# ithewei/libhv

Hardware: AMD Instinct MI355X
Metric: device-resident WS unmask GiB/s, 64 KiB masked frames, 1/2/4/8 MI355X (higher is better)
Workload: dtype u8

## Files before the change

### libhv_amd/csrc/hvws_utf8.hip

```cpp
#include "hvws_dev.h"

namespace hvws {

namespace {

constexpr int U8_T = 256, U8_U = 4;
static_assert((uint64_t)U8_T * U8_U * 16u == U8_TILE, "tile geometry");
constexpr int U8_MAXF = 512;

__device__ __forceinline__ uint32_t u8_step(uint32_t s, uint32_t b) {
    if (s == 0u) {
        if (b < 0x80u) return 0u;
        if (b < 0xC2u) return U8_REJECT;
        if (b < 0xE0u) return 1u;
        if (b == 0xE0u) return 3u;
        if (b == 0xEDu) return 4u;
        if (b < 0xF0u) return 2u;
        if (b == 0xF0u) return 5u;
        if (b < 0xF4u) return 6u;
        return b == 0xF4u ? 7u : U8_REJECT;
    }
    if (s > 7u) return U8_REJECT;
    const uint32_t lo = s == 3u ? 0xA0u : (s == 5u ? 0x90u : 0x80u);
    const uint32_t hi = s == 4u ? 0x9Fu : (s == 7u ? 0x8Fu : 0xBFu);
    if (b < lo || b > hi) return U8_REJECT;
    return s == 1u ? 0u : (s <= 4u ? 1u : 2u);
}

__device__ __forceinline__ uint32_t u8_len(uint32_t b) {
    return b < 0x80u ? 1u : b < 0xC0u ? 0u : b < 0xC2u ? 9u : b < 0xE0u ? 2u : b < 0xF0u ? 3u : b < 0xF5u ? 4u : 9u;
}

__device__ __forceinline__ bool u8_ok2(uint32_t p, uint32_t q) {
    const uint32_t lo = p == 0xE0u ? 0xA0u : (p == 0xF0u ? 0x90u : 0x80u);
    const uint32_t hi = p == 0xEDu ? 0x9Fu : (p == 0xF4u ? 0x8Fu : 0xBFu);
    return q >= lo && q <= hi;
}

__device__ __forceinline__ bool u8_chunk_bad(const u32x4 w, const uint32_t h, const uint32_t jlo,
                                             const uint32_t jhi) {
    if (((w.x | w.y | w.z | w.w | (h >> 8)) & 0x80808080u) == 0u) return false;
    {
        auto top4 = [](uint32_t x) { return (((x >> 7) & 0x01010101u) * 0x01020408u) >> 24; };
        const uint32_t hb = (top4(h) >> 1) | (top4(w.x) << 3) | (top4(w.y) << 7) | (top4(w.z) << 11) | (top4(w.w) << 15);
        const uint32_t reads = ((1u << (jhi + 3u)) - 1u) & ~((1u << jlo) - 1u);
        if ((hb & reads) == 0u) return false;
    }
    uint32_t B[19], L[19];
    B[0] = (h >> 8) & 0xFFu;
    B[1] = (h >> 16) & 0xFFu;
    B[2] = h >> 24;
    const uint32_t ww[4] = {w.x, w.y, w.z, w.w};
#pragma unroll
    for (int q = 0; q < 16; ++q) B[3 + q] = (ww[q >> 2] >> (8 * (q & 3))) & 0xFFu;
#pragma unroll
    for (int q = 0; q < 19; ++q) L[q] = u8_len(B[q]);
    bool P[18];
#pragma unroll
    for (int q = 0; q < 18; ++q) P[q] = u8_ok2(B[q], B[q + 1]);
    uint32_t badm = 0u;
#pragma unroll
    for (int j = 0; j < 16; ++j) {
        const uint32_t l0 = L[j + 3], l1 = L[j + 2], l2 = L[j + 1], l3 = L[j];
        bool ok;
        if (l0 == 0u)
            ok = l1 != 0u ? (l1 >= 2u && l1 <= 4u && P[j + 2])
               : l2 != 0u ? (l2 >= 3u && l2 <= 4u && P[j + 1])
               : l3 != 0u ? (l3 == 4u && P[j])
                          : false;
        else
            ok = l0 != 9u && (l1 != 0u ? l1 == 1u : l2 != 0u ? l2 == 2u : l3 != 0u ? (l3 == 3u && P[j]) : true);
        badm |= ok ? 0u : (1u << j);
    }
    const uint32_t act = (jhi >= 16u ? 0xFFFFu : ((1u << jhi) - 1u)) & ~((1u << jlo) - 1u);
    return (badm & act) != 0u;
}

__device__ __forceinline__ void u8_report(bool bad, uint32_t rec, uint32_t* __restrict__ flags) {
    uint64_t m = __ballot(bad);
    const uint32_t lane = threadIdx.x & 63u;
    while (m) {
        const int l = __ffsll((unsigned long long)m) - 1;
        const uint32_t r = (uint32_t)__shfl((int)rec, l);
        const uint64_t same = __ballot(bad && rec == r);
        if (lane == (uint32_t)l) atomicOr(&flags[r], 1u);
        m &= ~same;
    }
}

template <typename OFF, typename END, typename KEY>
__device__ __forceinline__ void u8_chunk(const u32x4 v, const uint32_t h, const uint64_t c, const uint32_t k0,
                                         const uint32_t nf, OFF offf, END endf, KEY keyf, bool& bad, uint32_t& brec,
                                         uint32_t* __restrict__ flags) {
    uint32_t lo = 0, hi = nf;
    while (lo < hi) {
        const uint32_t mid = (lo + hi) >> 1;
        if (endf(mid) > c) hi = mid;
        else lo = mid + 1;
    }
#pragma unroll 1
    for (uint32_t k = lo; k < nf; ++k) {
        const uint64_t o = offf(k), e = endf(k);
        if (o >= c + 16) break;
        const uint64_t from = o + 3 > c ? o + 3 - c : 0;
        const uint32_t jlo = from > 16 ? 16u : (uint32_t)from;
        const uint32_t jhi = e < c + 16 ? (e > c ? (uint32_t)(e - c) : 0u) : 16u;
        if (jlo < jhi) {
            const uint32_t kw = keyf(k);
            if (u8_chunk_bad(v ^ u32x4{kw, kw, kw, kw}, h ^ kw, jlo, jhi)) {
                if (!bad) {
                    bad = true;
                    brec = k0 + k;
                } else if (brec != k0 + k) {
                    atomicOr(&flags[k0 + k], 1u);
                }
            }
        }
        if (e > c + 16) break;
    }
}

__global__ __launch_bounds__(U8_T) void k_u8_tiles(const uint8_t* __restrict__ rx, uint64_t rx_len,
                                                   const uint64_t* __restrict__ pay_off,
                                                   const uint64_t* __restrict__ pay_len,
                                                   const uint32_t* __restrict__ keyrot,
                                                   const uint32_t* __restrict__ tile_first,
                                                   const uint64_t* __restrict__ nfr_p, uint64_t cap, uint32_t masked,
                                                   uint32_t* __restrict__ flags) {
    constexpr int T = U8_T, U = U8_U;
    __shared__ uint64_t s_off[U8_MAXF];
    __shared__ uint64_t s_end[U8_MAXF];
    __shared__ uint32_t s_key[U8_MAXF];

    const uint64_t t = blockIdx.x;
    const uint64_t base = t * U8_TILE;
    const uint32_t tid = threadIdx.x;
    const uint64_t nfr = *nfr_p < cap ? *nfr_p : cap;
    const uint32_t k0 = tile_first[t];
    const uint32_t k1r = tile_first[t + 1];
    const uint32_t k1 = (uint64_t)k1r + 1 < nfr ? k1r + 1 : (uint32_t)nfr;
    const uint32_t nf = k1 > k0 ? k1 - k0 : 0u;
    if (nf == 0u) return;

    const bool full = base + U8_TILE <= rx_len;
    u32x4 v[U];
    uint32_t h[U];
#pragma unroll
    for (int i = 0; i < U; ++i) {
        const uint64_t c = base + ((uint64_t)i * T + tid) * 16u;
        if (full || c + 16 <= rx_len) {
            v[i] = *reinterpret_cast<const u32x4*>(rx + c);
        } else {
            uint32_t w[4] = {0u, 0u, 0u, 0u};
            for (int b = 0; b < 16; ++b)
                if (c + b < rx_len) w[b >> 2] |= (uint32_t)rx[c + b] << (8 * (b & 3));
            v[i] = u32x4{w[0], w[1], w[2], w[3]};
        }
    }
#pragma unroll
    for (int i = 0; i < U; ++i) {
        const uint64_t c = base + ((uint64_t)i * T + tid) * 16u;
        uint32_t prev = (uint32_t)__shfl_up((int)v[i].w, 1);
        if ((tid & 63u) == 0u) prev = (c >= 16 && c <= rx_len) ? *reinterpret_cast<const uint32_t*>(rx + c - 4) : 0u;
        h[i] = prev;
    }

    const bool staged = nf <= (uint32_t)U8_MAXF;
    if (staged) {
        for (uint32_t i = tid; i < nf; i += T) {
            const uint64_t o = pay_off[k0 + i], n = pay_len[k0 + i];
            s_off[i] = o;
            s_end[i] = n > 6 ? o + n : o;
            s_key[i] = masked ? keyrot[k0 + i] : 0u;
        }
    }
    __syncthreads();

#pragma unroll
    for (int i = 0; i < U; ++i) {
        const uint64_t c = base + ((uint64_t)i * T + tid) * 16u;
        bool bad = false;
        uint32_t brec = 0u;
        if (c < rx_len) {
            if (staged)
                u8_chunk(
                    v[i], h[i], c, k0, nf, [&](uint32_t k) { return s_off[k]; }, [&](uint32_t k) { return s_end[k]; },
                    [&](uint32_t k) { return s_key[k]; }, bad, brec, flags);
            else
                u8_chunk(
                    v[i], h[i], c, k0, nf, [&](uint32_t k) { return pay_off[k0 + k]; },
                    [&](uint32_t k) {
                        const uint64_t n = pay_len[k0 + k];
                        return n > 6 ? pay_off[k0 + k] + n : pay_off[k0 + k];
                    },
                    [&](uint32_t k) { return masked ? keyrot[k0 + k] : 0u; }, bad, brec, flags);
        }
        u8_report(bad, brec, flags);
    }
}

__global__ __launch_bounds__(256) void k_u8_words(const uint8_t* __restrict__ rx, uint64_t rx_len,
                                                  const uint64_t* __restrict__ pay_off,
                                                  const uint64_t* __restrict__ pay_len,
                                                  const uint32_t* __restrict__ keyrot,
                                                  const uint64_t* __restrict__ nfr_p, uint64_t cap, uint32_t masked,
                                                  uint32_t* __restrict__ flags, uint32_t* __restrict__ words,
                                                  uint64_t* __restrict__ meta) {
    const uint64_t nfr = *nfr_p < cap ? *nfr_p : cap;
    const uint64_t k = (uint64_t)blockIdx.x * blockDim.x + threadIdx.x;
    if (k == 0) meta[0] = nfr;
    if (k >= nfr) return;
    const uint64_t o = pay_off[k], n = pay_len[k];
    const uint32_t kw = masked ? keyrot[k] : 0u;
    const uint32_t interior_bad = flags[k];
    if (interior_bad) flags[k] = 0u;
    if (o > rx_len || n > rx_len - o) {
        words[k] = 0xFFFFFFFFu;
        return;
    }
    auto byte_at = [&](uint64_t i) -> uint32_t {
        const uint64_t a = o + i;
        return ((uint32_t)rx[a] ^ (kw >> (8u * (uint32_t)(a & 3u)))) & 0xFFu;
    };
    uint32_t word = 0u;
    if (n <= 6) {
        uint32_t d[6];
#pragma unroll
        for (int i = 0; i < 6; ++i) d[i] = (uint64_t)i < n ? byte_at(i) : 0u;
#pragma unroll
        for (uint32_t e = 0; e < 8; ++e) {
            uint32_t s = e;
#pragma unroll
            for (int i = 0; i < 6; ++i)
                if ((uint64_t)i < n) s = u8_step(s, d[i]);
            word |= s << (4u * e);
        }
    } else {
        const uint32_t d0 = byte_at(0), d1 = byte_at(1), d2 = byte_at(2);
        const uint32_t t0 = byte_at(n - 3), t1 = byte_at(n - 2), t2 = byte_at(n - 1);
        uint32_t tail = 0u;
        if (u8_len(t2) != 0u) tail = u8_step(0u, t2);
        else if (u8_len(t1) != 0u) tail = u8_step(u8_step(0u, t1), t2);
        else if (u8_len(t0) != 0u) tail = u8_step(u8_step(u8_step(0u, t0), t1), t2);
#pragma unroll
        for (uint32_t e = 0; e < 8; ++e) {
            const uint32_t s = u8_step(u8_step(u8_step(e, d0), d1), d2);
            word |= ((s == U8_REJECT || interior_bad) ? U8_REJECT : tail) << (4u * e);
        }
    }
    words[k] = word;
}

__device__ __forceinline__ void u8_apply(uint32_t& st, uint32_t& text, uint32_t inf, uint32_t w) {
    const uint32_t op = inf & F_OPMASK;
    if (op >= 3u) return;
    if ((inf & I_HDR) && op == 1u) {
        text = 1u;
        st = U8_ACCEPT;
    } else if ((inf & I_HDR) && op == 2u) {
        text = 0u;
        st = U8_ACCEPT;
    }
    if (text && (inf & I_BODY)) st = st > 7u ? U8_REJECT : (w >> (4u * st)) & 15u;
    if ((inf & I_END) && (inf & F_FIN) && text) {
        if (st != U8_ACCEPT) st = U8_REJECT;
        text = 0u;
    }
}

__global__ __launch_bounds__(256) void k_u8_fold(const uint32_t* __restrict__ info, const uint32_t* __restrict__ words,
                                                 const uint64_t* __restrict__ meta,
                                                 const uint64_t* __restrict__ counts,
                                                 const uint64_t* __restrict__ bases, uint32_t nseg,
                                                 const uint32_t* __restrict__ state_in,
                                                 uint32_t* __restrict__ state_out, uint64_t* __restrict__ bad_out) {
    const uint32_t s = __builtin_amdgcn_readfirstlane(blockIdx.x * (blockDim.x >> 6) + (threadIdx.x >> 6));
    if (s >= nseg) return;
    const uint32_t lane = threadIdx.x & 63u;
    const uint64_t nrec = meta[0];
    const uint64_t first = bases[s];
    uint64_t cnt = counts[s];
    if (first >= nrec) cnt = 0;
    else if (cnt > nrec - first) cnt = nrec - first;
    const uint32_t sw = state_in ? state_in[s] : 0u;
    uint32_t st = sw & 15u, text = (sw >> 4) & 1u;
    uint64_t bad = ~0ull;
    if (st > 7u) {
        st = U8_REJECT;
        bad = first;
        cnt = 0;
    }
    for (uint64_t b0 = 0; b0 < cnt && bad == ~0ull; b0 += 64) {
        const uint64_t left = cnt - b0;
        const uint32_t m = left < 64 ? (uint32_t)left : 64u;
        const uint32_t my_info = lane < m ? info[first + b0 + lane] : 8u;
        const uint32_t my_word = lane < m ? words[first + b0 + lane] : U8_IDENTITY;
        const uint32_t op = my_info & F_OPMASK;
        const bool reset = (my_info & I_HDR) && (op == 1u || op == 2u);
        const uint64_t below = __ballot(reset) & ((2ull << lane) - 1ull);
        const uint32_t r = below ? 63u - (uint32_t)__clzll((long long)below) : 0u;
        uint32_t lst = below ? U8_ACCEPT : st, ltext = below ? 0u : text;
        const uint32_t span = lane < m ? lane - r : 0u;
        for (uint32_t t = 0;; ++t) {
            const bool act = lane < m && t <= span;
            if (!__ballot(act)) break;
            const uint32_t src = r + t < 64u ? r + t : 63u;
            const uint32_t inf = (uint32_t)__shfl((int)my_info, (int)src);
            const uint32_t w = (uint32_t)__shfl((int)my_word, (int)src);
            if (act) u8_apply(lst, ltext, inf, w);
        }
        const uint64_t rej = __ballot(lane < m && lst == U8_REJECT);
        if (rej) {
            st = U8_REJECT;
            bad = first + b0 + (uint64_t)(__ffsll((unsigned long long)rej) - 1);
        } else {
            st = (uint32_t)__builtin_amdgcn_readlane((int)lst, (int)(m - 1u));
            text = (uint32_t)__builtin_amdgcn_readlane((int)ltext, (int)(m - 1u));
        }
    }
    if (st == U8_REJECT) text = 0u;
    if (lane == 0u) {
        state_out[s] = st | (text << 4);
        bad_out[s] = bad;
    }
}

}

hipError_t launch_utf8(const uint8_t* rx, uint64_t rx_len, const uint64_t* pay_off, const uint64_t* pay_len,
                       const uint32_t* keyrot, const uint32_t* info, const uint64_t* nfr_dev, uint64_t cap,
                       const uint32_t* tile_first, uint64_t ntiles, int masked, uint32_t* flags, uint32_t* words,
                       uint64_t* meta, const uint64_t* counts, const uint64_t* bases, uint32_t nseg,
                       const uint32_t* state_in, uint32_t* state_out, uint64_t* bad, hipStream_t st) {
    if (ntiles)
        hipLaunchKernelGGL(k_u8_tiles, dim3((uint32_t)ntiles), dim3(U8_T), 0, st, rx, rx_len, pay_off, pay_len, keyrot,
                           tile_first, nfr_dev, cap, masked ? 1u : 0u, flags);
    const uint64_t wb = (cap + 255) / 256;
    hipLaunchKernelGGL(k_u8_words, dim3((uint32_t)(wb ? wb : 1)), dim3(256), 0, st, rx, rx_len, pay_off, pay_len, keyrot,
                       nfr_dev, cap, masked ? 1u : 0u, flags, words, meta);
    if (nseg)
        hipLaunchKernelGGL(k_u8_fold, dim3((nseg + 3) / 4), dim3(256), 0, st, info, words, meta, counts, bases, nseg,
                           state_in, state_out, bad);
    return hipGetLastError();
}

}
```

Baseline: 3017.

## Replace per-byte UTF-8 check with SWAR predicate and single-frame fast path

Swaps the scalar 19-byte UTF-8 validation inside u8_chunk_bad for a SWAR bitwise classifier that works on whole 32-bit words, using alignbyte to shift across word boundaries. It also adds an early path for tiles that sit entirely inside one frame's payload: the XOR key is applied and every chunk is checked without staging frame metadata in shared memory or searching records. Both aim to cut ALU work and per-tile bookkeeping on the validation kernel. The cost is a complex, hard-to-verify bit-trick predicate that must match the reference exactly, and the early return skips the __syncthreads path for the whole block.

Result: slower. 2811 (-6.8%).

```diff
diff --git a/libhv_amd/csrc/hvws_u8_pred.h b/libhv_amd/csrc/hvws_u8_pred.h
--- /dev/null
+++ b/libhv_amd/csrc/hvws_u8_pred.h
@@ -0,0 +1,117 @@
+#pragma once
+#include <stdint.h>
+
+#if defined(__HIPCC__)
+#define HVWS_U8_FN __host__ __device__ __forceinline__
+#else
+#define HVWS_U8_FN inline
+#endif
+
+namespace hvws {
+
+HVWS_U8_FN uint32_t u8_len(uint32_t b) {
+    return b < 0x80u ? 1u : b < 0xC0u ? 0u : b < 0xC2u ? 9u : b < 0xE0u ? 2u : b < 0xF0u ? 3u : b < 0xF5u ? 4u : 9u;
+}
+
+HVWS_U8_FN bool u8_ok2(uint32_t p, uint32_t q) {
+    const uint32_t lo = p == 0xE0u ? 0xA0u : (p == 0xF0u ? 0x90u : 0x80u);
+    const uint32_t hi = p == 0xEDu ? 0x9Fu : (p == 0xF4u ? 0x8Fu : 0xBFu);
+    return q >= lo && q <= hi;
+}
+
+HVWS_U8_FN uint32_t u8_pred_ref(uint32_t w0, uint32_t w1, uint32_t w2, uint32_t w3, uint32_t h) {
+    uint32_t B[19], L[19];
+    B[0] = (h >> 8) & 0xFFu;
+    B[1] = (h >> 16) & 0xFFu;
+    B[2] = h >> 24;
+    const uint32_t ww[4] = {w0, w1, w2, w3};
+#pragma unroll
+    for (int q = 0; q < 16; ++q) B[3 + q] = (ww[q >> 2] >> (8 * (q & 3))) & 0xFFu;
+#pragma unroll
+    for (int q = 0; q < 19; ++q) L[q] = u8_len(B[q]);
+    bool P[18];
+#pragma unroll
+    for (int q = 0; q < 18; ++q) P[q] = u8_ok2(B[q], B[q + 1]);
+    uint32_t badm = 0u;
+#pragma unroll
+    for (int j = 0; j < 16; ++j) {
+        const uint32_t l0 = L[j + 3], l1 = L[j + 2], l2 = L[j + 1], l3 = L[j];
+        bool ok;
+        if (l0 == 0u)
+            ok = l1 != 0u ? (l1 >= 2u && l1 <= 4u && P[j + 2])
+               : l2 != 0u ? (l2 >= 3u && l2 <= 4u && P[j + 1])
+               : l3 != 0u ? (l3 == 4u && P[j])
+                          : false;
+        else
+            ok = l0 != 9u && (l1 != 0u ? l1 == 1u : l2 != 0u ? l2 == 2u : l3 != 0u ? (l3 == 3u && P[j]) : true);
+        badm |= ok ? 0u : (1u << j);
+    }
+    return badm;
+}
+
+HVWS_U8_FN uint32_t u8_bytes_from(uint32_t hi, uint32_t lo, uint32_t n) {
+#if defined(__HIP_DEVICE_COMPILE__)
+    return __builtin_amdgcn_alignbyte(hi, lo, n);
+#else
+    return (lo >> (8u * n)) | (hi << (32u - 8u * n));
+#endif
+}
+
+struct U8Cls {
+    uint32_t cc, w1, w2, w3, c, z;
+};
+
+HVWS_U8_FN U8Cls u8_classes(uint32_t x, uint32_t nx) {
+    constexpr uint32_t M = 0x80808080u, ONE = 0x01010101u;
+    const uint32_t y = x & 0x7F7F7F7Fu;
+    const uint32_t gC2 = y + 0x3Eu * ONE, gE0 = y + 0x20u * ONE, gE1 = y + 0x1Fu * ONE, gED = y + 0x13u * ONE,
+                   gEE = y + 0x12u * ONE, gF0 = y + 0x10u * ONE, gF1 = y + 0x0Fu * ONE, gF4 = y + 0x0Cu * ONE,
+                   gF5 = y + 0x0Bu * ONE;
+    const uint32_t n5 = nx << 2, n45 = n5 | (nx << 3);
+    const uint32_t e0 = gE0 & ~gE1, ed = gED & ~gEE, f0 = gF0 & ~gF1, f4 = gF4 & ~gF5;
+    const uint32_t fl = ((ed & n5) | (e0 & ~n5)) | ((f4 & n45) | (f0 & ~n45));
+    const uint32_t nf = x & ~(gF5 | fl);
+    const uint32_t u1 = nf & gC2, u2 = nf & gE0, u3 = nf & gF0;
+    const uint32_t xr = x >> 1;
+    const uint32_t c = x & ~(x << 1);
+    const uint32_t c6 = xr & ~x;
+    const uint32_t v3 = (u2 & ~gF0) | c;
+    const uint32_t l2 = x & gC2 & ~gE0;
+    U8Cls k;
+    k.cc = (c & M) | (c6 & ~M);
+    k.w1 = (u1 & M) | (~xr & ~M);
+    k.w2 = (u2 & M) | ((l2 >> 1) & ~M);
+    k.w3 = (u3 & M) | ((v3 >> 1) & ~M);
+    k.c = c;
+    k.z = x & ~(gC2 & ~gF5);
+    return k;
+}
+
+HVWS_U8_FN void u8_pred_flags(uint32_t w0, uint32_t w1, uint32_t w2, uint32_t w3, uint32_t h, uint32_t bad[4]) {
+    constexpr uint32_t M = 0x80808080u;
+    const uint32_t x[5] = {h, w0, w1, w2, w3};
+    U8Cls k[5];
+#pragma unroll
+    for (int i = 0; i < 5; ++i) k[i] = u8_classes(x[i], u8_bytes_from(i < 4 ? x[i + 1] : 0u, x[i], 1));
+    uint32_t y2[5], y1[5];
+#pragma unroll
+    for (int i = 0; i < 5; ++i) y2[i] = k[i].w2 | (k[i].cc & u8_bytes_from(k[i].w3, i ? k[i - 1].w3 : 0u, 3));
+#pragma unroll
+    for (int i = 0; i < 5; ++i) y1[i] = k[i].w1 | (k[i].cc & u8_bytes_from(y2[i], i ? y2[i - 1] : 0u, 3));
+#pragma unroll
+    for (int i = 1; i < 5; ++i) {
+        const uint32_t r = u8_bytes_from(y1[i], y1[i - 1], 3);
+        bad[i - 1] = M & ~((k[i].c & r) | ((r << 1) & ~k[i].z));
+    }
+}
+
+HVWS_U8_FN uint32_t u8_pred(uint32_t w0, uint32_t w1, uint32_t w2, uint32_t w3, uint32_t h) {
+    uint32_t bad[4];
+    u8_pred_flags(w0, w1, w2, w3, h, bad);
+    uint32_t r = 0u;
+#pragma unroll
+    for (int i = 0; i < 4; ++i) r |= (((bad[i] >> 7) * 0x01020408u) >> 24) << (4 * i);
+    return r;
+}
+
+}
diff --git a/libhv_amd/csrc/hvws_utf8.hip b/libhv_amd/csrc/hvws_utf8.hip
--- a/libhv_amd/csrc/hvws_utf8.hip
+++ b/libhv_amd/csrc/hvws_utf8.hip
@@ -1,4 +1,5 @@
 #include "hvws_dev.h"
+#include "hvws_u8_pred.h"
 
 namespace hvws {
 
@@ -27,16 +28,6 @@
     return s == 1u ? 0u : (s <= 4u ? 1u : 2u);
 }
 
-__device__ __forceinline__ uint32_t u8_len(uint32_t b) {
-    return b < 0x80u ? 1u : b < 0xC0u ? 0u : b < 0xC2u ? 9u : b < 0xE0u ? 2u : b < 0xF0u ? 3u : b < 0xF5u ? 4u : 9u;
-}
-
-__device__ __forceinline__ bool u8_ok2(uint32_t p, uint32_t q) {
-    const uint32_t lo = p == 0xE0u ? 0xA0u : (p == 0xF0u ? 0x90u : 0x80u);
-    const uint32_t hi = p == 0xEDu ? 0x9Fu : (p == 0xF4u ? 0x8Fu : 0xBFu);
-    return q >= lo && q <= hi;
-}
-
 __device__ __forceinline__ bool u8_chunk_bad(const u32x4 w, const uint32_t h, const uint32_t jlo,
                                              const uint32_t jhi) {
     if (((w.x | w.y | w.z | w.w | (h >> 8)) & 0x80808080u) == 0u) return false;
@@ -46,32 +37,7 @@
         const uint32_t reads = ((1u << (jhi + 3u)) - 1u) & ~((1u << jlo) - 1u);
         if ((hb & reads) == 0u) return false;
     }
-    uint32_t B[19], L[19];
-    B[0] = (h >> 8) & 0xFFu;
-    B[1] = (h >> 16) & 0xFFu;
-    B[2] = h >> 24;
-    const uint32_t ww[4] = {w.x, w.y, w.z, w.w};
-#pragma unroll
-    for (int q = 0; q < 16; ++q) B[3 + q] = (ww[q >> 2] >> (8 * (q & 3))) & 0xFFu;
-#pragma unroll
-    for (int q = 0; q < 19; ++q) L[q] = u8_len(B[q]);
-    bool P[18];
-#pragma unroll
-    for (int q = 0; q < 18; ++q) P[q] = u8_ok2(B[q], B[q + 1]);
-    uint32_t badm = 0u;
-#pragma unroll
-    for (int j = 0; j < 16; ++j) {
-        const uint32_t l0 = L[j + 3], l1 = L[j + 2], l2 = L[j + 1], l3 = L[j];
-        bool ok;
-        if (l0 == 0u)
-            ok = l1 != 0u ? (l1 >= 2u && l1 <= 4u && P[j + 2])
-               : l2 != 0u ? (l2 >= 3u && l2 <= 4u && P[j + 1])
-               : l3 != 0u ? (l3 == 4u && P[j])
-                          : false;
-        else
-            ok = l0 != 9u && (l1 != 0u ? l1 == 1u : l2 != 0u ? l2 == 2u : l3 != 0u ? (l3 == 3u && P[j]) : true);
-        badm |= ok ? 0u : (1u << j);
-    }
+    const uint32_t badm = u8_pred(w.x, w.y, w.z, w.w, h);
     const uint32_t act = (jhi >= 16u ? 0xFFFFu : ((1u << jhi) - 1u)) & ~((1u << jlo) - 1u);
     return (badm & act) != 0u;
 }
@@ -163,6 +129,18 @@
         uint32_t prev = (uint32_t)__shfl_up((int)v[i].w, 1);
         if ((tid & 63u) == 0u) prev = (c >= 16 && c <= rx_len) ? *reinterpret_cast<const uint32_t*>(rx + c - 4) : 0u;
         h[i] = prev;
+    }
+
+    if (nf == 1u && full) {
+        const uint64_t o = pay_off[k0], n = pay_len[k0];
+        if (n > 6 && o + 3 <= base && base + U8_TILE <= o + n) {
+            const uint32_t kw = masked ? keyrot[k0] : 0u;
+            bool bad = false;
+#pragma unroll
+            for (int i = 0; i < U; ++i) bad |= u8_chunk_bad(v[i] ^ u32x4{kw, kw, kw, kw}, h[i] ^ kw, 0u, 16u);
+            if (__ballot(bad) && (tid & 63u) == 0u) atomicOr(&flags[k0], 1u);
+            return;
+        }
     }
 
     const bool staged = nf <= (uint32_t)U8_MAXF;
```
